# telegraphroad/VCNF

Measured on AMD Instinct MI355X. Metric: flow transforms/sec (log_prob + sample), D=64 RQ-spline, batch=1M, higher is better.
Workload: dtype f32 results on fp16x3 split operands: every fp32 operand of a conditioner GEMM travels as hi + lo fp16 halves, three f16 matrix instructions per product (four in the 48- and 16-deep layers), fp32 accumulation; measured against fp64 (tests/test_gpu_gemm_error.py): GEMM error 0.6-0.75x the exact-fp32

## Files before the change

### vcnf_amd/csrc/fused_layer_v6.hip

```cpp
#include <hip/hip_runtime.h>
#include <stdint.h>

#include "../../include/vcnf_hip.h"
#include "rqs_math.hpp"
#include "fused_common.hpp"
#include "host_common.hpp"
#include "rqs_lean.hpp"
#include "split_half.hpp"

#ifndef VCNF_ABL
#define VCNF_ABL 0
#endif
#ifndef VCNF_TIME
#define VCNF_TIME 0
#endif
#ifndef VCNF_AHEAD
#define VCNF_AHEAD 1
#endif
#if VCNF_TIME
#define VCNF_T(I) { const long long t_ = clock64(); tacc[I] += t_ - tlast; tlast = t_; }
#define VCNF_TIME_PARAM , float* tstamps
#define VCNF_TIME_ARG , time_buffer()
#else
#define VCNF_T(I)
#define VCNF_TIME_PARAM
#define VCNF_TIME_ARG
#endif

#define VCNF_SYNC() { __builtin_amdgcn_sched_barrier(0); asm volatile("s_waitcnt lgkmcnt(0)\n\ts_barrier" ::: "memory"); __builtin_amdgcn_sched_barrier(0); }

namespace vcnf {

#if VCNF_TIME
constexpr int kTimeSlots = 24;
static float* time_buffer() {
  static float* buf = nullptr;
  if (!buf && hipMalloc(&buf, 2 * kTimeSlots * sizeof(float)) != hipSuccess) buf = nullptr;
  return buf;
}
extern "C" int vcnf_v6_phase_stamps(float* out) {
  if (!time_buffer() || hipDeviceSynchronize() != hipSuccess) return VCNF_ERR_LAUNCH;
  return hipMemcpy(out, time_buffer(), 2 * kTimeSlots * sizeof(float), hipMemcpyDeviceToHost) == hipSuccess ? VCNF_OK : VCNF_ERR_LAUNCH;
}
#endif

template <int DI, int DT, int C, int H, int NBLK, int K, bool INV>
__global__ __launch_bounds__(512, 2) void fused_rqs_layer_v6_kernel(const FusedArgs a VCNF_TIME_PARAM) {
  static_assert(H == 128 && K == 8, "4 row blocks of 32 over 4 waves; 3 K - 1 = 23 logits: two features per 48 rows");
  static_assert((DI == 16 || DI == 32) && DT == DI && (C == 0 || C == 16), "shape family");
  constexpr int kBlock = 512;
  constexpr int kTile = 128;
  constexpr int NCB = 4;
  constexpr int D = DI + DT;
  constexpr int XS = D + 4;
  constexpr int NTX = DI / 16;
  constexpr int NTC = C / 16;
  constexpr int NT0 = NTX + NTC;
  constexpr int NTH = H / 16;
  constexpr int P = 3 * K - 1;
  constexpr int NG = DT / 4;
  constexpr int NR = NG / 2;
  constexpr int TABW = 3 * (K + 1);
  using L = PackLayout6<DI, DT, C, H, NBLK, K>;
  constexpr int GFRAG = 3 * NTH * 2 * 64;
  constexpr int RING = VCNF_AHEAD + 1;

  extern __shared__ __align__(16) float smem[];
  using S = LdsV6<DI, DT, C, H, NBLK, K>;
  static_assert(S::TILE == kTile && S::FRAG_N == 2 * GFRAG * 4 && S::XT_N == kTile * XS && S::TAB_N >= DI * TABW, "layout");
  uint4* act = reinterpret_cast<uint4*>(smem + S::FRAG);
  uint4* act_hi = act;
  uint4* act_lo = act + NTH * NCB * 64;
  float* xt = smem + S::XT;
  uint4* ctxf = reinterpret_cast<uint4*>(smem + S::CTXF);
  float* tab = smem + S::TAB;
  float* ldt = smem + S::LDT;
  int* tfi = reinterpret_cast<int*>(smem + S::TFI);
  int* idi = reinterpret_cast<int*>(smem + S::IDI);
  constexpr int NBV = C > 0 ? 3 : 2;
  constexpr int NBT = S::NBT;
  constexpr int BPL = S::BPL;
  float* biasf = smem + S::BIAS;
  float* ldold = smem + S::LDOLD;
  int* tflag = reinterpret_cast<int*>(smem + S::TFLAG);

  const int tid = threadIdx.x;
  const int lane = tid & 63;
  const int wave = __builtin_amdgcn_readfirstlane(tid >> 6);
  const int rp = wave & 3;
  const int ch = wave >> 2;
  const int c32 = lane & 31;
  const int kg = lane >> 5;
  const RqsConst& c = a.c;
  const bool shared = a.sh_w != nullptr;
  const LeanConst lc = make_lean_const(c);

  if (ch == 1) __builtin_amdgcn_s_setprio(1);
  for (int i = tid; i < NG * 96; i += kBlock) {
    const int g = i / 96, hf = i % 96 / 48;
    biasf[hf * BPL + g * 48 + i % 48] = a.wpack[L::BF + i];
  }
  for (int i = tid; i < NBT * H; i += kBlock) {
    const int v = i / H, blk = (v - 1) / NBV, sel = (v - 1) % NBV, r = i % H;
    const int off = v == 0 ? L::B0 : L::BLK0 + blk * L::BLK + (sel == 0 ? L::BA : sel == 1 ? L::BB : L::BC);
    biasf[(r >> 4 & 1) * BPL + NG * 48 + v * (H / 2) + (r >> 5) * 16 + (r & 15)] = a.wpack[off + r];
  }
  for (int i = tid; i < DT; i += kBlock) tfi[i] = a.tf_idx[i];
  for (int i = tid; i < DI; i += kBlock) idi[i] = a.id_idx[i];
  if (shared) {
    for (int i = tid; i < 3 * DI; i += kBlock) {
      const int f = i % DI;
      SplitLogits p{a.sh_w + f * K, a.sh_h + f * K, a.sh_d + f * (K - 1), K, 1.f, c.edge_logit, c.tails};
      rqs_build_table_part_k<K>(p, c, tab + f * TABW, 1, i / DI);
    }
  }

  const __amdgpu_buffer_rsrc_t wr =
      __builtin_amdgcn_make_buffer_rsrc(const_cast<float*>(a.wpack), 0, a.wpack_bytes, 0x00020000);
  const int voff = lane * 16;
  const float* bplane = biasf + kg * BPL;

  const long long ntiles = (a.B + kTile - 1) / kTile;
  bool bad = false;
  float satm = 0.f;
#if VCNF_TIME
  long long tacc[20], tlast = clock64();
  const long long tstart = tlast, rstart = wall_clock64();
  for (int i = 0; i < 20; ++i) tacc[i] = 0;
#endif
  float4 xpre[kTile * (D / 4) / kBlock], cpre[1];
  static_assert(kTile * (D / 4) % kBlock == 0 && (C == 0 || kTile * (C / 4) == kBlock), "rows per thread");
#define VCNF_PREFETCH_ROWS(TILE)                                                          \
  {                                                                                       \
    const long long pb0 = min((TILE) * kTile, a.B);                                       \
    const long long left = (a.B - pb0) * (D * 4);                                         \
    const __amdgpu_buffer_rsrc_t xr_ = __builtin_amdgcn_make_buffer_rsrc(                 \
        const_cast<float*>(a.x) + pb0 * D, 0, (int)min(left, (long long)(kTile * D * 4)), 0x00020000); \
    _Pragma("unroll") for (int k = 0; k < kTile * (D / 4) / kBlock; ++k)                  \
      xpre[k] = __builtin_bit_cast(float4, __builtin_amdgcn_raw_buffer_load_b128(xr_, (tid + kBlock * k) * 16, 0, 0)); \
    if (C > 0) {                                                                          \
      const long long leftc = (a.B - pb0) * (C * 4);                                      \
      const __amdgpu_buffer_rsrc_t cr_ = __builtin_amdgcn_make_buffer_rsrc(               \
          const_cast<float*>(a.ctx) + pb0 * C, 0, (int)min(leftc, (long long)(kTile * C * 4)), 0x00020000); \
      cpre[0] = __builtin_bit_cast(float4, __builtin_amdgcn_raw_buffer_load_b128(cr_, tid * 16, 0, 0)); \
    }                                                                                     \
  }
#define VCNF_ROWS_ARRIVED()                                                               \
  {                                                                                       \
    _Pragma("unroll") for (int k = 0; k < kTile * (D / 4) / kBlock; ++k) {                \
      floatx4 v_ = __builtin_bit_cast(floatx4, xpre[k]);                                  \
      asm volatile("" : "+v"(v_));                                                        \
      xpre[k] = __builtin_bit_cast(float4, v_);                                           \
    }                                                                                     \
    if (C > 0) {                                                                          \
      floatx4 v_ = __builtin_bit_cast(floatx4, cpre[0]);                                  \
      asm volatile("" : "+v"(v_));                                                        \
      cpre[0] = __builtin_bit_cast(float4, v_);                                           \
    }                                                                                     \
  }
  VCNF_PREFETCH_ROWS((long long)blockIdx.x)
  VCNF_ROWS_ARRIVED()
  for (long long tile = blockIdx.x; tile < ntiles; tile += gridDim.x) {
    const long long b0 = tile * kTile;
    const int rows = (int)min((long long)kTile, a.B - b0);
    satm = 0.f;
    { VCNF_T(0) VCNF_SYNC(); VCNF_T(15) }
    {
      constexpr int D4 = D / 4;
      if (tid == 0) *tflag = 0;
#pragma unroll
      for (int k = 0; k < kTile * D4 / kBlock; ++k) {
        const int i = tid + kBlock * k;
        const int r = i / D4, o = i - r * D4;
        *reinterpret_cast<float4*>(xt + r * XS + 4 * o) = xpre[k];
      }
      if (C > 0) {
        const int r = tid >> 2, part = tid & 3;
        half4 h4, l4;
        const float cv[4] = {cpre[0].x, cpre[0].y, cpre[0].z, cpre[0].w};
#pragma unroll
        for (int i = 0; i < 4; ++i) satm = fmaxf(satm, cv[i] == cv[i] ? __builtin_fabsf(cv[i]) : __builtin_inff());
        asm volatile("" : "+v"(satm));
#pragma unroll
        for (int i = 0; i < 4; ++i) {
          const float x = __builtin_amdgcn_fmed3f(cv[i], -65504.f, 65504.f);
          const _Float16 hv = (_Float16)x;
          h4[i] = hv;
          l4[i] = (_Float16)((x - (float)hv) * kLoScale);
        }
        const int at = (((r >> 5) * 2) * 64 + (r & 31) + 32 * (part >> 1));
        uint2* dh = reinterpret_cast<uint2*>(ctxf + at) + (part & 1);
        uint2* dl = reinterpret_cast<uint2*>(ctxf + at + 64) + (part & 1);
        *dh = __builtin_bit_cast(uint2, h4);
        *dl = __builtin_bit_cast(uint2, l4);
      }
    }
    { VCNF_T(1) VCNF_SYNC(); VCNF_T(15) }

    {
      constexpr int UNR = DI / 4;
      const int mi = tid >> 2, part = tid & 3;
      float lsum = 0.f;
      float xv[UNR], fv[UNR];
      float* px[UNR];
#pragma unroll
      for (int k = 0; k < UNR; ++k) {
        px[k] = xt + mi * XS + idi[part * UNR + k];
        xv[k] = *px[k];
        fv[k] = xv[k];
      }
      if (shared) {
        float yv[UNR], lad[UNR];
        bool in_[UNR];
#pragma unroll
        for (int k = 0; k < UNR; ++k) {
          in_[k] = (xv[k] >= c.lo_x) && (xv[k] <= c.hi_x);
          bool bad1 = false;
          rqs_point_table_inside<INV, K>(in_[k] ? xv[k] : c.lo_x, tab + (part * UNR + k) * TABW, yv[k], lad[k], bad1);
          bad = bad || (bad1 && in_[k]);
        }
#pragma unroll
        for (int k = 0; k < UNR; ++k) {
          const float o = in_[k] ? yv[k] : xv[k];
          *px[k] = o;
          if (INV) fv[k] = o;
          lsum += in_[k] ? lad[k] : 0.f;
        }
      }
      lsum += __shfl_xor(lsum, 1, 64);
      lsum += __shfl_xor(lsum, 2, 64);
      int tid_ = tid;
      asm volatile("" : "+v"(tid_));
      if (part == 0) ldt[tid_ >> 2] = lsum;
#pragma unroll
      for (int k = 0; k < UNR; ++k) satm = fmaxf(satm, fv[k] == fv[k] ? 0.f : __builtin_inff());
      const int k0 = part * UNR;
      const int t0 = k0 >> 4, kg0 = (k0 >> 3) & 1;
      const int at = (t0 * NCB + (mi >> 5)) * 64 + (mi & 31) + 32 * kg0;
      if (UNR == 8) {
        half8 h8, l8;
        float f8[8];
#pragma unroll
        for (int k = 0; k < 8; ++k) f8[k] = fv[k < UNR ? k : 0];
        split8<false>(f8, h8, l8, satm);
        act_hi[at] = __builtin_bit_cast(uint4, h8);
        act_lo[at] = __builtin_bit_cast(uint4, l8);
      } else {
        half4 h4, l4;
        satm = fmaxf(fmaxf(satm, __builtin_fabsf(fv[0])), __builtin_fabsf(fv[1]));
        satm = fmaxf(fmaxf(satm, __builtin_fabsf(fv[2 < UNR ? 2 : 0])), __builtin_fabsf(fv[3 < UNR ? 3 : 0]));
        asm volatile("" : "+v"(satm));
#pragma unroll
        for (int i = 0; i < 4; ++i) {
          const float x = __builtin_amdgcn_fmed3f(fv[i < UNR ? i : 0], -65504.f, 65504.f);
          const _Float16 hv = (_Float16)x;
          h4[i] = hv;
          l4[i] = (_Float16)((x - (float)hv) * kLoScale);
        }
        reinterpret_cast<uint2*>(act_hi + at)[(k0 >> 2) & 1] = __builtin_bit_cast(uint2, h4);
        reinterpret_cast<uint2*>(act_lo + at)[(k0 >> 2) & 1] = __builtin_bit_cast(uint2, l4);
      }
    }
    { VCNF_T(2) VCNF_SYNC(); VCNF_T(15) }
    if (ch == 1) { VCNF_T(14) VCNF_SYNC(); VCNF_T(16) }

    half8 ahi[NTH], alo[NTH];
    floatx16 abias;
#define VCNF_LOAD_BIAS16(DST, VEC)                                                        \
  _Pragma("unroll") for (int i_ = 0; i_ < 4; ++i_) {                                      \
    const floatx4 b4_ = *reinterpret_cast<const floatx4*>(bplane + NG * 48 + (VEC) * (H / 2) + 16 * rp + 4 * i_); \
    DST[4 * i_ + 0] = b4_[0]; DST[4 * i_ + 1] = b4_[1]; DST[4 * i_ + 2] = b4_[2]; DST[4 * i_ + 3] = b4_[3]; \
  }
#define VCNF_LOAD_HIDDEN(WOFF, BVEC)                                                      \
  {                                                                                       \
    _Pragma("unroll") for (int t = 0; t < NTH; ++t) {                                     \
      ahi[t] = __builtin_bit_cast(half8, wload(wr, voff, 4 * ((WOFF) + ((rp * NTH + t) * 2 + 0) * 256))); \
      alo[t] = __builtin_bit_cast(half8, wload(wr, voff, 4 * ((WOFF) + ((rp * NTH + t) * 2 + 1) * 256))); \
    }                                                                                     \
    VCNF_LOAD_BIAS16(abias, BVEC)                                                         \
  }

    floatx16 h[2];
    {
      half8 w0h[NT0], w0l[NT0];
      floatx16 bias0;
#pragma unroll
      for (int t = 0; t < NT0; ++t) {
        w0h[t] = __builtin_bit_cast(half8, wload(wr, voff, 4 * (L::W0 + ((rp * NT0 + t) * 2 + 0) * 256)));
        w0l[t] = __builtin_bit_cast(half8, wload(wr, voff, 4 * (L::W0 + ((rp * NT0 + t) * 2 + 1) * 256)));
      }
      VCNF_LOAD_BIAS16(bias0, 0)
#pragma unroll
      for (int j = 0; j < 2; ++j) {
        const int cb = 2 * ch + j;
        floatx16 mainv = bias0, corr = {}, corr2 = {};
#pragma unroll
        for (int t = 0; t < NT0; ++t) {
          const half8 bh = __builtin_bit_cast(half8, t < NTX ? act_hi[(t * NCB + cb) * 64 + lane] : ctxf[(cb * 2 + 0) * 64 + lane]);
          const half8 bl = __builtin_bit_cast(half8, t < NTX ? act_lo[(t * NCB + cb) * 64 + lane] : ctxf[(cb * 2 + 1) * 64 + lane]);
          mainv = mfma32h(w0h[t], bh, mainv);
          corr = mfma32h(w0h[t], bl, corr);
          corr = mfma32h(w0l[t], bh, corr);
          corr2 = mfma32h(w0l[t], bl, corr2);
        }
#pragma unroll
        for (int r = 0; r < 16; ++r) h[j][r] = fmaf(fmaf(corr2[r], kLoUnscale, corr[r]), kLoUnscale, mainv[r]);
      }
    }
    { VCNF_T(3) VCNF_SYNC(); VCNF_T(15) }
#define VCNF_PUBLISH(SRC, RELU)                                                           \
  _Pragma("unroll") for (int j = 0; j < 2; ++j) {                                         \
    _Pragma("unroll") for (int hh = 0; hh < 2; ++hh) {                                    \
      float v8_[8];                                                                       \
      _Pragma("unroll") for (int i = 0; i < 8; ++i) v8_[i] = SRC[j][8 * hh + i];          \
      half8 h8_, l8_;                                                                     \
      split8<RELU>(v8_, h8_, l8_, satm);                                                  \
      const int at = ((2 * rp + hh) * NCB + 2 * ch + j) * 64 + lane;                      \
      act_hi[at] = __builtin_bit_cast(uint4, h8_);                                        \
      act_lo[at] = __builtin_bit_cast(uint4, l8_);                                        \
    }                                                                                     \
  }
    VCNF_LOAD_HIDDEN(L::BLK0 + L::WA, 1)
    VCNF_PUBLISH(h, true)
    { VCNF_T(4) VCNF_SYNC(); VCNF_T(15) }

#define VCNF_READ_B(T)                                                                    \
  {                                                                                       \
    rh[(T) % RING] = __builtin_bit_cast(half8, act_hi[((((T) & 7)) * NCB + 2 * ch + ((T) >> 3)) * 64 + lane]); \
    rl[(T) % RING] = __builtin_bit_cast(half8, act_lo[((((T) & 7)) * NCB + 2 * ch + ((T) >> 3)) * 64 + lane]); \
  }
#define VCNF_HIDDEN_COMPUTE(OUT)                                                          \
  {                                                                                       \
    half8 rh[RING], rl[RING];                 \
    floatx16 corr;                                                                        \
    _Pragma("unroll") for (int st_ = 0; st_ < VCNF_AHEAD; ++st_) {                        \
      VCNF_READ_B(st_)                                                                    \
    }                                                                                     \
    _Pragma("unroll") for (int st_ = 0; st_ < 2 * NTH; ++st_) {                           \
      const int j = st_ >> 3, tk_ = st_ & 7;                                              \
      if (st_ + VCNF_AHEAD < 2 * NTH) {                                                   \
        VCNF_READ_B(st_ + VCNF_AHEAD)                                                     \
      }                                                                                   \
      if (tk_ == 0) {                                                                       \
        OUT[j] = abias;                                                                   \
        corr = floatx16{};                                                                \
      }                                                                                   \
      OUT[j] = mfma32h(ahi[tk_], rh[st_ % RING], OUT[j]);                                      \
      corr = mfma32h(ahi[tk_], rl[st_ % RING], corr);                                          \
      corr = mfma32h(alo[tk_], rh[st_ % RING], corr);                                          \
      if (tk_ == NTH - 1) {                                                                 \
        _Pragma("unroll") for (int r = 0; r < 16; ++r) OUT[j][r] = fmaf(corr[r], kLoUnscale, OUT[j][r]); \
      }                                                                                   \
    }                                                                                     \
    __builtin_amdgcn_sched_group_barrier(0x100, 2 * VCNF_AHEAD, 0);                       \
    _Pragma("unroll") for (int st_ = 0; st_ + VCNF_AHEAD < 2 * NTH; ++st_) {              \
      __builtin_amdgcn_sched_group_barrier(0x100, 2, 0);                                  \
      __builtin_amdgcn_sched_group_barrier(0x008, 3, 0);                                  \
    }                                                                                     \
    __builtin_amdgcn_sched_group_barrier(0x008, 3 * VCNF_AHEAD, 0);                       \
  }

#pragma unroll
    for (int blk = 0; blk < (VCNF_ABL == 5 ? 0 : NBLK); ++blk) {
      const int base = L::BLK0 + blk * L::BLK;
      floatx16 t[2];
      VCNF_HIDDEN_COMPUTE(t)
      { VCNF_T(5) VCNF_SYNC(); VCNF_T(15) }
      VCNF_LOAD_HIDDEN(base + L::WB, 2 + blk * NBV)
      half8 wch, wcl;
      floatx16 gate[2], gbias;
      if (C > 0) {
        wch = __builtin_bit_cast(half8, wload(wr, voff, 4 * (base + L::WC + (rp * 2 + 0) * 256)));
        wcl = __builtin_bit_cast(half8, wload(wr, voff, 4 * (base + L::WC + (rp * 2 + 1) * 256)));
        VCNF_LOAD_BIAS16(gbias, 3 + blk * NBV)
      }
      VCNF_PUBLISH(t, true)
      { VCNF_T(6) VCNF_SYNC(); VCNF_T(15) }
      VCNF_HIDDEN_COMPUTE(t)
      if (C > 0 && VCNF_ABL != 6) {
#pragma unroll
        for (int j = 0; j < 2; ++j) {
          const half8 bh = __builtin_bit_cast(half8, ctxf[((2 * ch + j) * 2 + 0) * 64 + lane]);
          const half8 bl = __builtin_bit_cast(half8, ctxf[((2 * ch + j) * 2 + 1) * 64 + lane]);
          floatx16 corr = {}, corr2 = {};
          gate[j] = mfma32h(wch, bh, gbias);
          corr = mfma32h(wch, bl, corr);
          corr = mfma32h(wcl, bh, corr);
          corr2 = mfma32h(wcl, bl, corr2);
#pragma unroll
          for (int r = 0; r < 16; ++r) gate[j][r] = fmaf(fmaf(corr2[r], kLoUnscale, corr[r]), kLoUnscale, gate[j][r]);
        }
      }
      { VCNF_T(5) VCNF_SYNC(); VCNF_T(15) }
      if (blk + 1 < NBLK) {
        VCNF_LOAD_HIDDEN(base + L::BLK + L::WA, 1 + (blk + 1) * NBV)
      }
      if (C > 0 && VCNF_ABL != 6) {
#pragma unroll
        for (int j = 0; j < 2; ++j) {
#pragma unroll
          for (int r = 0; r < 16; ++r) {
            const float sg = hw_rcp(1.f + hw_exp2(-gate[j][r]));
            h[j][r] = fmaf(t[j][r], sg, h[j][r]);
          }
        }
      } else {
#pragma unroll
        for (int j = 0; j < 2; ++j) h[j] += t[j];
      }
      if (blk + 1 < NBLK) {
        VCNF_PUBLISH(h, true)
      } else {
        VCNF_PUBLISH(h, false)
      }
      { VCNF_T(7) VCNF_SYNC(); VCNF_T(15) }
    }
    if (ch == 0) { VCNF_T(14) VCNF_SYNC(); VCNF_T(17) }
#undef VCNF_HIDDEN_COMPUTE
#undef VCNF_READ_B
#undef VCNF_LOAD_HIDDEN
#undef VCNF_PUBLISH

    half8 fhi[NTH], flo[NTH];
#pragma unroll
    for (int t = 0; t < NTH; ++t) {
      fhi[t] = __builtin_bit_cast(half8, act_hi[(t * NCB + rp) * 64 + lane]);
      flo[t] = __builtin_bit_cast(half8, act_lo[(t * NCB + rp) * 64 + lane]);
    }
    float ld_acc = 0.f;
    uint4* win = act + ch * GFRAG;
    const int gtid = tid & 255;
    constexpr int NSTG = GFRAG / 256;
    static_assert(GFRAG % 256 == 0, "whole fragments per thread");
#define VCNF_STAGE_DMA(G)                                                                 \
  _Pragma("unroll") for (int k = 0; k < NSTG; ++k)                                        \
    dma16_to_lds(wr, win + (gtid & ~63) + k * 256, gtid * 16, 4 * (L::WF + (G) * (4 * GFRAG) + k * 1024));
    floatx16 pa[3];
#define VCNF_LOAD_BIASF(G)                                                                \
  _Pragma("unroll") for (int b = 0; b < 3; ++b) {                                         \
    _Pragma("unroll") for (int i_ = 0; i_ < 4; ++i_) {                                    \
      const floatx4 b4_ = *reinterpret_cast<const floatx4*>(bplane + (G) * 48 + 16 * b + 4 * i_); \
      pa[b][4 * i_ + 0] = b4_[0]; pa[b][4 * i_ + 1] = b4_[1]; pa[b][4 * i_ + 2] = b4_[2]; pa[b][4 * i_ + 3] = b4_[3]; \
    }                                                                                     \
  }
    VCNF_LOAD_BIASF(ch)
    { VCNF_T(8) VCNF_SYNC(); VCNF_T(15) }
    VCNF_STAGE_DMA(ch)
    if (ch == 0 && rp < 2 && a.ld_mode) {
      const __amdgpu_buffer_rsrc_t or_ = __builtin_amdgcn_make_buffer_rsrc(a.logdet + b0, 0, rows * 4, 0x00020000);
      __builtin_amdgcn_raw_ptr_buffer_load_lds(or_, (__attribute__((address_space(3))) void*)(ldold + rp * 64), 4,
                                               lane * 4, rp * 256, 0, 0);
    }
    wait_vector_memory();
    { VCNF_T(9) VCNF_SYNC(); VCNF_T(15) }
    if (ch == 1) { VCNF_T(14) VCNF_SYNC(); VCNF_T(18) }
    for (int rnd = 0; rnd < (VCNF_ABL == 3 ? 0 : NR); ++rnd) {
      const int g = 2 * rnd + ch;
      float* px[2];
      float xin[2];
#pragma unroll
      for (int f2 = 0; f2 < 2; ++f2) {
        px[f2] = xt + (rp * 32 + c32) * XS + tfi[4 * g + 2 * kg + f2];
        xin[f2] = *px[f2];
      }
      {
        half8 wh[RING], wl[RING];
        floatx16 corr;
#define VCNF_READ_W(T)                                                                    \
  {                                                                                       \
    wh[(T) % RING] = __builtin_bit_cast(half8, win[((T) * 2 + 0) * 64 + lane]);           \
    wl[(T) % RING] = __builtin_bit_cast(half8, win[((T) * 2 + 1) * 64 + lane]);           \
  }
#pragma unroll
        for (int u = 0; u < VCNF_AHEAD; ++u) {
          VCNF_READ_W(u)
        }
#pragma unroll
        for (int u = 0; u < 3 * NTH; ++u) {
          const int b = u >> 3, t = u & 7;
          if (u + VCNF_AHEAD < 3 * NTH) {
            VCNF_READ_W(u + VCNF_AHEAD)
          }
          if (t == 0) corr = floatx16{};
          pa[b] = mfma32h(wh[u % RING], fhi[t], pa[b]);
          corr = mfma32h(wh[u % RING], flo[t], corr);
          corr = mfma32h(wl[u % RING], fhi[t], corr);
          if (t == NTH - 1) {
#pragma unroll
            for (int r = 0; r < 16; ++r) pa[b][r] = fmaf(corr[r], kLoUnscale, pa[b][r]);
          }
        }
        __builtin_amdgcn_sched_group_barrier(0x100, 2 * VCNF_AHEAD, 0);
#pragma unroll
        for (int u = 0; u + VCNF_AHEAD < 3 * NTH; ++u) {
          __builtin_amdgcn_sched_group_barrier(0x100, 2, 0);
          __builtin_amdgcn_sched_group_barrier(0x008, 3, 0);
        }
        __builtin_amdgcn_sched_group_barrier(0x008, 3 * VCNF_AHEAD, 0);
#undef VCNF_READ_W
      }
      { VCNF_T(10) VCNF_SYNC(); VCNF_T(15) }
      {
        const bool more = rnd + 1 < NR;
        if (!more) {
          VCNF_PREFETCH_ROWS(tile + gridDim.x)
        }
        if (more && VCNF_ABL != 2) {
          VCNF_STAGE_DMA(g + 2)
        }
        float yv[2], lad[2];
#pragma unroll
        for (int f2 = 0; f2 < 2; ++f2) {
          float lg[P];
#pragma unroll
          for (int tl = 0; tl < P; ++tl) lg[tl] = pa[(24 * f2 + tl) >> 4][(24 * f2 + tl) & 15];
          rqs_lean_eval<8, INV>(xin[f2], lg, lc, yv[f2], lad[f2], bad);
        }
        *px[0] = yv[0];
        *px[1] = yv[1];
        ld_acc += lad[0] + lad[1];
        if (more) {
          VCNF_LOAD_BIASF(g + 2)
        }
      }
      if (rnd + 1 < NR && VCNF_ABL != 2) wait_vector_memory();
      { VCNF_T(11) VCNF_SYNC(); VCNF_T(15) }
    }
    if (ch == 0) { VCNF_T(14) VCNF_SYNC(); VCNF_T(19) }
#undef VCNF_PREFETCH_ROWS
#undef VCNF_STAGE_DMA
#undef VCNF_LOAD_BIASF

    ld_acc += __shfl_xor(ld_acc, 32, 64);
    if (ch == 1 && kg == 0) ldt[rp * 32 + c32] += ld_acc;
    if (satm > 65504.f) *tflag = 1;
    { VCNF_T(12) VCNF_SYNC(); VCNF_T(15) }
    VCNF_ROWS_ARRIVED()
#undef VCNF_ROWS_ARRIVED
    int tid_ = tid;
    asm volatile("" : "+v"(tid_));
    const bool over = *tflag != 0;
    if (tid == 0 && over && a.sat) atomicAdd(a.sat, 1);
    if (a.redo) {
      if (tid_ < kTile / kFusedFlagRows) {
        const __amdgpu_buffer_rsrc_t rr = __builtin_amdgcn_make_buffer_rsrc(
            a.redo + tile * (kTile / kFusedFlagRows), 0, 4 * ((rows + kFusedFlagRows - 1) / kFusedFlagRows), 0x00020000);
        __builtin_amdgcn_raw_buffer_store_b32(over ? 1 : 0, rr, tid_ * 4, 0, 0);
      }
      if (over) continue;
    }
    if (ch == 0 && (tid_ & 32) == 0) {
      const int mrow = (tid_ >> 6) * 32 + (tid_ & 31);
      const __amdgpu_buffer_rsrc_t lr = __builtin_amdgcn_make_buffer_rsrc(a.logdet + b0, 0, rows * 4, 0x00020000);
      const float o = a.ld_sign * (ld_acc + ldt[mrow]);
      __builtin_amdgcn_raw_buffer_store_b32(__builtin_bit_cast(unsigned, a.ld_mode ? ldold[mrow] + o : o), lr, mrow * 4, 0, 0);
    }
    {
      constexpr int D4 = D / 4;
      const __amdgpu_buffer_rsrc_t yr = __builtin_amdgcn_make_buffer_rsrc(a.y + b0 * D, 0, rows * (D * 4), 0x00020000);
      floatx4 yv[kTile * D4 / kBlock];
#pragma unroll
      for (int k = 0; k < kTile * D4 / kBlock; ++k) {
        const int i = tid_ + kBlock * k;
        const int r = i / D4, o = i - r * D4;
        yv[k] = *reinterpret_cast<const floatx4*>(xt + r * XS + 4 * o);
      }
#pragma unroll
      for (int k = 0; k < kTile * D4 / kBlock; ++k)
        __builtin_amdgcn_raw_buffer_store_b128(__builtin_bit_cast(__attribute__((ext_vector_type(4))) unsigned, yv[k]), yr, (tid_ + kBlock * k) * 16, 0, 0);
    }
  }
#if VCNF_TIME
  VCNF_T(13)
  if (blockIdx.x == 0 && (tid & 255) == 0 && tstamps) {
    float* ts = tstamps + (tid >> 8) * kTimeSlots;
    for (int i = 0; i < 20; ++i) ts[i] = (float)tacc[i];
    ts[20] = (float)(clock64() - tstart);
    ts[21] = (float)(wall_clock64() - rstart);
    ts[22] = (float)((ntiles - blockIdx.x + gridDim.x - 1) / gridDim.x);
  }
#endif
  if (INV && a.bad && bad) atomicAdd(a.bad, 1);
}

template <int DI, int DT, int C, int H, int NBLK, int K>
static int launch_v6(const FusedArgs& a, int inverse, hipStream_t st) {
  constexpr int TILE = 128;
  constexpr size_t lds = LdsV6<DI, DT, C, H, NBLK, K>::BYTES;
  const bool set = inverse ? lds_limit_once<&fused_rqs_layer_v6_kernel<DI, DT, C, H, NBLK, K, true>>(lds)
                           : lds_limit_once<&fused_rqs_layer_v6_kernel<DI, DT, C, H, NBLK, K, false>>(lds);
  if (!set) return VCNF_ERR_LAUNCH;
  const long long ntiles = (a.B + TILE - 1) / TILE;
  dim3 grid((unsigned)(ntiles < 256 ? ntiles : 256));
  if (inverse)
    hipLaunchKernelGGL((fused_rqs_layer_v6_kernel<DI, DT, C, H, NBLK, K, true>), grid, dim3(512), lds, st, a VCNF_TIME_ARG);
  else
    hipLaunchKernelGGL((fused_rqs_layer_v6_kernel<DI, DT, C, H, NBLK, K, false>), grid, dim3(512), lds, st, a VCNF_TIME_ARG);
  return launched();
}

template <int NBLK>
static int launch_v6_family(const FusedArgs& a, int d_id, int ctx_dim, int inverse, hipStream_t st) {
#ifdef VCNF_DEV_ONLY
  return launch_v6<32, 32, 16, 128, NBLK, 8>(a, inverse, st);
#else
  return with_fused_shape(d_id, ctx_dim,
                          [&](auto DI, auto C) { return launch_v6<DI(), DI(), C(), 128, NBLK, 8>(a, inverse, st); });
#endif
}

#ifndef VCNF_V6_NBLK
#define VCNF_V6_NBLK 2
#endif
VCNF_BLOCKS_ENTRY(launch_fused_v6_b, VCNF_V6_NBLK, FusedArgs, launch_v6_family)

}
```

### vcnf_amd/csrc/fused_lds.hpp

```cpp
#pragma once

#include <stddef.h>

namespace vcnf {

template <int DI, int DT, int C, int H, int NBLK, int K>
struct LdsV6 {
  static constexpr int TILE = 128, D = DI + DT, NG = DT / 4;
  static constexpr int NBT = 1 + NBLK * (C > 0 ? 3 : 2);
  static constexpr int BPL = NG * 48 + NBT * (H / 2);
  static constexpr int FRAG = 0, FRAG_N = 2 * 3 * (H / 16) * 2 * 64 * 4;
  static constexpr int XT = FRAG + FRAG_N, XT_N = TILE * (D + 4);
  static constexpr int CTXF = XT + XT_N, CTXF_N = C > 0 ? 4 * 2 * 64 * 4 : 0;
  static constexpr int TAB = CTXF + CTXF_N, TAB_N = (DI * 3 * (K + 1) + 3) & ~3;
  static constexpr int LDT = TAB + TAB_N, LDT_N = TILE;
  static constexpr int TFI = LDT + LDT_N, TFI_N = DT;
  static constexpr int IDI = TFI + TFI_N, IDI_N = DI + 4;
  static constexpr int BIAS = IDI + IDI_N, BIAS_N = 2 * BPL;
  static constexpr int LDOLD = BIAS + BIAS_N, LDOLD_N = TILE;
  static constexpr int TFLAG = LDOLD + LDOLD_N, TFLAG_N = 1;
  static constexpr int END = TFLAG + TFLAG_N;
  static constexpr size_t SLACK_BYTES = 3 * 4 + 64;
  static constexpr size_t BYTES = (size_t)END * 4 + SLACK_BYTES;
  static_assert(FRAG == 0 && FRAG + FRAG_N <= XT && XT + XT_N <= CTXF && CTXF + CTXF_N <= TAB && TAB + TAB_N <= LDT &&
                    LDT + LDT_N <= TFI && TFI + TFI_N <= IDI && IDI + IDI_N <= BIAS && BIAS + BIAS_N <= LDOLD &&
                    LDOLD + LDOLD_N <= TFLAG && (size_t)(TFLAG + TFLAG_N) * 4 <= BYTES,
                "regions in order, none overlaps the next, the last ends within BYTES");
  static_assert(XT % 4 == 0 && CTXF % 4 == 0 && TAB % 4 == 0, "16-byte aligned rows and fragments");
};

template <int DI, int DT, int C, int H, int NBLK, int K>
struct LdsV6s {
  static constexpr int TILE = 32, D = DI + DT, NG = DT / 4;
  static constexpr int TABF = (DI * 3 * (K + 1) + 3) & ~3;
  static constexpr int TSET = TABF + DT + DI + 4 + NG * 96;
  static constexpr int ACT = 0, ACT_N = 4 * (H / 16) * 64 * 4;
  static constexpr int XT = ACT + ACT_N, XT_N = TILE * (D + 4);
  static constexpr int CTXF = XT + XT_N, CTXF_N = C > 0 ? 2 * 64 * 4 : 0;
  static constexpr int LDT = CTXF + CTXF_N, LDT_N = TILE;
  static constexpr int LDX = LDT + LDT_N, LDX_N = 8 * TILE;
  static constexpr int TFLAG = LDX + LDX_N, TFLAG_N = 4;
  static constexpr int TSETS = TFLAG + TFLAG_N, TSETS_N = 2 * TSET;
  static constexpr int END = TSETS + TSETS_N;
  static constexpr size_t SLACK_BYTES = 64;
  static constexpr size_t BYTES = (size_t)END * 4 + SLACK_BYTES;
  static_assert(ACT == 0 && ACT + ACT_N <= XT && XT + XT_N <= CTXF && CTXF + CTXF_N <= LDT && LDT + LDT_N <= LDX &&
                    LDX + LDX_N <= TFLAG && TFLAG + TFLAG_N <= TSETS && (size_t)(TSETS + TSETS_N) * 4 <= BYTES,
                "regions in order, none overlaps the next, the last ends within BYTES");
  static_assert(XT % 4 == 0 && CTXF % 4 == 0 && TSETS % 4 == 0 && TSET % 4 == 0, "16-byte aligned rows and tables");
};

template <int DI, int DT, int C, int H, int NBLK, int K, int kCB>
struct LdsF32 {
  static constexpr int TILE = 4 * kCB * 16, D = DI + DT;
  static constexpr int XT = 0, XT_N = TILE * (D + 4);
  static constexpr int CT = XT + XT_N, CT_N = TILE * ((C > 0 ? C : 4) + 4);
  static constexpr int TAB = CT + CT_N, TAB_N = (DI * 3 * (K + 1) + 3) & ~3;
  static constexpr int TFI = TAB + TAB_N, TFI_N = DT;
  static constexpr int IDI = TFI + TFI_N, IDI_N = DI;
  static constexpr int END = IDI + IDI_N;
  static constexpr size_t SLACK_BYTES = 64;
  static constexpr size_t BYTES = (size_t)END * 4 + SLACK_BYTES;
  static_assert(XT + XT_N <= CT && CT + CT_N <= TAB && TAB + TAB_N <= TFI && TFI + TFI_N <= IDI &&
                    (size_t)(IDI + IDI_N) * 4 <= BYTES,
                "regions in order, none overlaps the next, the last ends within BYTES");
  static_assert(CT % 4 == 0 && TAB % 4 == 0, "16-byte aligned rows");
};

}
```

### vcnf_amd/csrc/rqs_math.hpp

```cpp
#pragma once
#include <hip/hip_runtime.h>
#include <math.h>

#include "rqs_host.hpp"

#pragma clang fp contract(off)

namespace vcnf {

constexpr float kLog2e = 1.44269504088896340736f;
constexpr float kLn2 = 0.69314718055994530942f;
__device__ __forceinline__ float hw_exp2(float v) { return __builtin_amdgcn_exp2f(v); }
__device__ __forceinline__ float hw_rcp(float v) { return __builtin_amdgcn_rcpf(v); }
__device__ __forceinline__ float hw_log(float v) { return __builtin_amdgcn_logf(v) * kLn2; }
__device__ __forceinline__ float hw_sqrt(float v) { return __builtin_amdgcn_sqrtf(v); }
__device__ __forceinline__ float div_nr(float a, float b) {
  const float r = hw_rcp(b);
  const float q = a * r;
  return fmaf(fmaf(-b, q, a), r, q);
}

__device__ __forceinline__ float softplus_f(float v) {
  const float e = hw_exp2(v * kLog2e);
  const float u = 1.f + e;
  const float um1 = u - 1.f;
  const float l = (um1 == 0.f) ? e : hw_log(u) * div_nr(e, um1);
  return v > 20.f ? v : l;
}

__device__ __forceinline__ float rqs_rounding_level_zero(float disc, float qb, float p) {
  const float scale = fmaf(qb, qb, __builtin_fabsf(p));
  return (disc < 0.f && disc >= -6.103515625e-5f * scale) ? 0.f : disc;
}

struct RqsBin {
  float xl, w, yl, h, d0, d1;
};

template <bool INV>
__device__ __forceinline__ void rqs_bin_eval(float x, const RqsBin& b, float& y, float& lad, bool& bad) {
  const float s = div_nr(b.h, b.w);
  const float e = fmaf(-2.f, s, b.d0 + b.d1);
  if (!INV) {
    const float t = div_nr(x - b.xl, b.w);
    const float omt = 1.f - t;
    const float tt = t * omt;
    const float num = b.h * fmaf(s * t, t, b.d0 * tt);
    const float den = fmaf(e, tt, s);
    y = b.yl + div_nr(num, den);
    const float dn = (s * s) * fmaf(b.d1 * t, t, fmaf(2.f * s, tt, (b.d0 * omt) * omt));
    lad = fmaf(-2.f, hw_log(den), hw_log(dn));
  } else {
    const float dy = x - b.yl;
    const float qa = fmaf(dy, e, b.h * (s - b.d0));
    const float qb = fmaf(-dy, e, b.h * b.d0);
    const float qc = -s * dy;
    const float fa = 4.f * qa;
    const float p = fa * qc;
    const float perr = fmaf(fa, qc, -p);
    const float disc = rqs_rounding_level_zero(fmaf(qb, qb, -p) - perr, qb, p);
    bad = bad || !(disc >= 0.f);
    float r = div_nr(2.f * qc, -qb - hw_sqrt(disc));
    r = (dy <= b.h && r > 1.f) ? 1.f : r;
    y = fmaf(r, b.w, b.xl);
    const float omr = 1.f - r;
    const float rr = r * omr;
    const float den = fmaf(e, rr, s);
    const float dn = (s * s) * fmaf(b.d1 * r, r, fmaf(2.f * s, rr, (b.d0 * omr) * omr));
    lad = fmaf(2.f, hw_log(den), -hw_log(dn));
  }
}

template <int KT, bool INV, class P>
__device__ __forceinline__ void rqs_select(float x, const P& p, const RqsConst& c, float sc2, RqsBin& sel) {
  const int K = KT > 0 ? KT : c.K;
  constexpr int KR = KT > 0 ? KT : 1;
  float ew[KR], eh[KR];
  float mw = -INFINITY, mh = -INFINITY;
#pragma unroll
  for (int k = 0; k < K; ++k) {
    mw = fmaxf(mw, p.w(k));
    mh = fmaxf(mh, p.h(k));
  }
  float sw = 0.f, sh = 0.f;
#pragma unroll
  for (int k = 0; k < K; ++k) {
    const float a = hw_exp2((p.w(k) - mw) * sc2), b = hw_exp2((p.h(k) - mh) * sc2);
    if (KT > 0) { ew[k] = a; eh[k] = b; }
    sw += a;
    sh += b;
  }
  const float gw = div_nr(c.free_w, sw), gh = div_nr(c.free_h, sh);
  float cw = 0.f, ch = 0.f;
  float xl = c.lo_x, yl = c.lo_y, dl = p.d(0);
  sel.xl = xl; sel.yl = yl; sel.w = 1.f; sel.h = 1.f; sel.d0 = dl; sel.d1 = dl;
#pragma unroll
  for (int k = 0; k < K; ++k) {
    const float a = KT > 0 ? ew[k] : hw_exp2((p.w(k) - mw) * sc2);
    const float b = KT > 0 ? eh[k] : hw_exp2((p.h(k) - mh) * sc2);
    cw += fmaf(a, gw, c.min_w);
    ch += fmaf(b, gh, c.min_h);
    const float xr = (k == K - 1) ? c.hi_x : fmaf(c.span_x, cw, c.lo_x);
    const float yr = (k == K - 1) ? c.hi_y : fmaf(c.span_y, ch, c.lo_y);
    const float dr = p.d(k + 1);
    const bool take = (k == 0) || (INV ? (x >= yl) : (x >= xl));
    if (take) {
      sel.xl = xl; sel.w = xr - xl;
      sel.yl = yl; sel.h = yr - yl;
      sel.d0 = dl; sel.d1 = dr;
    }
    xl = xr; yl = yr; dl = dr;
  }
  sel.d0 = c.min_d + softplus_f(sel.d0);
  sel.d1 = c.min_d + softplus_f(sel.d1);
}

template <int K, bool INV>
struct RqsStaged {
  float ew[K], eh[K];
  float mw, mh, sw, sh, gw, gh, cw, ch, xl, yl, dl;
  RqsBin sel;
  template <class P>
  __device__ __forceinline__ void maxima(const P& p) {
    mw = -INFINITY;
    mh = -INFINITY;
#pragma unroll
    for (int k = 0; k < K; ++k) {
      mw = fmaxf(mw, p.w(k));
      mh = fmaxf(mh, p.h(k));
    }
    sw = 0.f;
    sh = 0.f;
  }
  template <class P>
  __device__ __forceinline__ void exps(const P& p, float sc2, int k0, int k1) {
#pragma unroll
    for (int k = 0; k < K; ++k) {
      if (k >= k0 && k < k1) {
        ew[k] = hw_exp2((p.w(k) - mw) * sc2);
        eh[k] = hw_exp2((p.h(k) - mh) * sc2);
        sw += ew[k];
        sh += eh[k];
      }
    }
  }
  template <class P>
  __device__ __forceinline__ void normalise(const P& p, const RqsConst& c) {
    gw = div_nr(c.free_w, sw);
    gh = div_nr(c.free_h, sh);
    cw = 0.f;
    ch = 0.f;
    xl = c.lo_x;
    yl = c.lo_y;
    dl = p.d(0);
    sel.xl = xl; sel.yl = yl; sel.w = 1.f; sel.h = 1.f; sel.d0 = dl; sel.d1 = dl;
  }
  template <class P>
  __device__ __forceinline__ void knots(float x, const P& p, const RqsConst& c, int k0, int k1) {
#pragma unroll
    for (int k = 0; k < K; ++k) {
      if (k < k0 || k >= k1) continue;
      cw += fmaf(ew[k], gw, c.min_w);
      ch += fmaf(eh[k], gh, c.min_h);
      const float xr = (k == K - 1) ? c.hi_x : fmaf(c.span_x, cw, c.lo_x);
      const float yr = (k == K - 1) ? c.hi_y : fmaf(c.span_y, ch, c.lo_y);
      const float dr = p.d(k + 1);
      const bool take = (k == 0) || (INV ? (x >= yl) : (x >= xl));
      sel.xl = take ? xl : sel.xl;
      sel.w = take ? xr - xl : sel.w;
      sel.yl = take ? yl : sel.yl;
      sel.h = take ? yr - yl : sel.h;
      sel.d0 = take ? dl : sel.d0;
      sel.d1 = take ? dr : sel.d1;
      xl = xr; yl = yr; dl = dr;
    }
  }
  __device__ __forceinline__ void derivatives(const RqsConst& c) {
    sel.d0 = c.min_d + softplus_f(sel.d0);
    sel.d1 = c.min_d + softplus_f(sel.d1);
  }
};

template <int KT, bool INV, class P>
__device__ __forceinline__ void rqs_point(float x, const P& p, const RqsConst& c,
                                          float& y, float& lad, bool& bad) {
  if (c.tails != 0 && !((x >= c.lo_x) && (x <= c.hi_x))) {
    y = x;
    lad = 0.f;
    return;
  }
  RqsBin sel;
  rqs_select<KT, INV>(x, p, c, p.scale * kLog2e, sel);
  rqs_bin_eval<INV>(x, sel, y, lad, bad);
}

struct PackedLogits {
  const float* q;
  int K;
  float scale, edge;
  int tails;
  __device__ __forceinline__ float w(int k) const { return q[k]; }
  __device__ __forceinline__ float h(int k) const { return q[K + k]; }
  __device__ __forceinline__ float d(int k) const {
    if (tails == 1) return (k == 0 || k == K) ? edge : q[2 * K + k - 1];
    if (tails == 2) return q[2 * K + (k == K ? 0 : k)];
    return q[2 * K + k];
  }
};

struct SplitLogits {
  const float *pw, *ph, *pd;
  int K;
  float scale, edge;
  int tails;
  __device__ __forceinline__ float w(int k) const { return pw[k]; }
  __device__ __forceinline__ float h(int k) const { return ph[k]; }
  __device__ __forceinline__ float d(int k) const {
    if (tails == 1) return (k == 0 || k == K) ? edge : pd[k - 1];
    if (tails == 2) return pd[k == K ? 0 : k];
    return pd[k];
  }
};

struct StridedLogits {
  const float *pw, *ph, *pd;
  long long ks;
  int K;
  float scale, edge;
  int tails;
  __device__ __forceinline__ float w(int k) const { return pw[k * ks]; }
  __device__ __forceinline__ float h(int k) const { return ph[k * ks]; }
  __device__ __forceinline__ float d(int k) const {
    if (tails == 1) return (k == 0 || k == K) ? edge : pd[(k - 1) * ks];
    if (tails == 2) return pd[(k == K ? 0 : k) * ks];
    return pd[k * ks];
  }
};

template <class P>
__device__ __forceinline__ void rqs_build_table_part(const P& p, const RqsConst& c, float* tab, int stride, int part) {
  const int K = c.K;
  float* col = tab + part * (K + 1) * stride;
  if (part == 2) {
    for (int k = 0; k <= K; ++k) col[k * stride] = c.min_d + softplus_f(p.d(k));
    return;
  }
  const bool xs = part == 0;
  float m = -INFINITY;
  for (int k = 0; k < K; ++k) m = fmaxf(m, xs ? p.w(k) : p.h(k));
  const float sc2 = p.scale * kLog2e;
  float sum = 0.f;
  for (int k = 0; k < K; ++k) sum += hw_exp2(((xs ? p.w(k) : p.h(k)) - m) * sc2);
  const float g = div_nr(xs ? c.free_w : c.free_h, sum);
  const float mn = xs ? c.min_w : c.min_h, span = xs ? c.span_x : c.span_y, lo = xs ? c.lo_x : c.lo_y;
  float cum = 0.f;
  col[0] = lo;
  for (int k = 0; k < K; ++k) {
    cum += fmaf(hw_exp2(((xs ? p.w(k) : p.h(k)) - m) * sc2), g, mn);
    col[(k + 1) * stride] = (k == K - 1) ? (xs ? c.hi_x : c.hi_y) : fmaf(span, cum, lo);
  }
}

template <int K, class P>
__device__ __forceinline__ void rqs_table_column_load(const P& p, int part, float (&v)[K + 1]) {
#pragma unroll
  for (int k = 0; k <= K; ++k) v[k] = part == 2 ? p.d(k) : (k < K ? (part == 0 ? p.w(k) : p.h(k)) : 0.f);
}

template <int K>
__device__ __forceinline__ void rqs_table_column_build(const float (&v)[K + 1], float scale, const RqsConst& c, float* tab,
                                                       int stride, int part) {
  float* col = tab + part * (K + 1) * stride;
  if (part == 2) {
#pragma unroll
    for (int k = 0; k <= K; ++k) col[k * stride] = c.min_d + softplus_f(v[k]);
    return;
  }
  const bool xs = part == 0;
  float e[K];
  float m = -INFINITY;
#pragma unroll
  for (int k = 0; k < K; ++k) m = fmaxf(m, v[k]);
  const float sc2 = scale * kLog2e;
  float sum = 0.f;
#pragma unroll
  for (int k = 0; k < K; ++k) {
    e[k] = hw_exp2((v[k] - m) * sc2);
    sum += e[k];
  }
  const float g = div_nr(xs ? c.free_w : c.free_h, sum);
  const float mn = xs ? c.min_w : c.min_h, span = xs ? c.span_x : c.span_y, lo = xs ? c.lo_x : c.lo_y;
  float cum = 0.f;
  col[0] = lo;
#pragma unroll
  for (int k = 0; k < K; ++k) {
    cum += fmaf(e[k], g, mn);
    col[(k + 1) * stride] = (k == K - 1) ? (xs ? c.hi_x : c.hi_y) : fmaf(span, cum, lo);
  }
}

template <int K, class P>
__device__ __forceinline__ void rqs_build_table_part_k(const P& p, const RqsConst& c, float* tab, int stride, int part) {
  float v[K + 1];
  rqs_table_column_load<K>(p, part, v);
  rqs_table_column_build<K>(v, p.scale, c, tab, stride, part);
}

template <class P>
__device__ __forceinline__ void rqs_build_table(const P& p, const RqsConst& c, float* tab, int stride = 1) {
#pragma unroll 1
  for (int part = 0; part < 3; ++part) rqs_build_table_part(p, c, tab, stride, part);
}

template <bool INV, int KT = 0>
__device__ __forceinline__ void rqs_point_table(float x, const float* tab, const RqsConst& c,
                                                float& y, float& lad, bool& bad) {
  if (c.tails != 0 && !((x >= c.lo_x) && (x <= c.hi_x))) {
    y = x;
    lad = 0.f;
    return;
  }
  const int K = KT > 0 ? KT : c.K;
  const float* xk = tab;
  const float* yk = tab + (K + 1);
  const float* dk = tab + 2 * (K + 1);
  int bin = 0;
  const float* key = INV ? yk : xk;
  if (KT > 0) {
#pragma unroll
    for (int k = 1; k < KT; ++k) bin += (x >= key[k]) ? 1 : 0;
  } else {
    for (int k = 1; k < K; ++k) bin += (x >= key[k]) ? 1 : 0;
  }
  RqsBin b;
  b.xl = xk[bin];
  b.w = xk[bin + 1] - b.xl;
  b.yl = yk[bin];
  b.h = yk[bin + 1] - b.yl;
  b.d0 = dk[bin];
  b.d1 = dk[bin + 1];
  rqs_bin_eval<INV>(x, b, y, lad, bad);
}

template <bool INV, int KT>
__device__ __forceinline__ void rqs_point_table_inside(float x, const float* tab, float& y, float& lad, bool& bad) {
  const float* xk = tab;
  const float* yk = tab + (KT + 1);
  const float* dk = tab + 2 * (KT + 1);
  const float* key = INV ? yk : xk;
  int bin = 0;
#pragma unroll
  for (int k = 1; k < KT; ++k) bin += (x >= key[k]) ? 1 : 0;
  RqsBin b;
  b.xl = xk[bin];
  b.w = xk[bin + 1] - b.xl;
  b.yl = yk[bin];
  b.h = yk[bin + 1] - b.yl;
  b.d0 = dk[bin];
  b.d1 = dk[bin + 1];
  rqs_bin_eval<INV>(x, b, y, lad, bad);
}

}
```

Before: 68.98 million.

## Precompute per-bin spline records in LDS and binary-search bins for shared RQS

Once per block, builds an 8-float record per spline bin (width reciprocal, slope, derivative terms, and inverse-quadratic coefficients) in an LDS region appended after the existing layout. The per-point evaluation then finds the bin with a branchless binary search across all unrolled points instead of a linear scan, loads the record with two float4 reads, and evaluates with fewer divides. The intent is to cut per-point ALU and LDS scalar loads in the shared-table spline stage. The cost is extra LDS per block, which may reduce occupancy, plus an added barrier and setup work at kernel start.

```diff
diff --git a/vcnf_amd/csrc/fused_layer_v6.hip b/vcnf_amd/csrc/fused_layer_v6.hip
--- a/vcnf_amd/csrc/fused_layer_v6.hip
+++ b/vcnf_amd/csrc/fused_layer_v6.hip
@@ -67,13 +67,15 @@
 
   extern __shared__ __align__(16) float smem[];
   using S = LdsV6<DI, DT, C, H, NBLK, K>;
-  static_assert(S::TILE == kTile && S::FRAG_N == 2 * GFRAG * 4 && S::XT_N == kTile * XS && S::TAB_N >= DI * TABW, "layout");
+  static_assert(S::TILE == kTile && S::FRAG_N == 2 * GFRAG * 4 && S::XT_N == kTile * XS && S::TAB_N >= DI * TABW &&
+                    S::BINS_PART == (DI / 4) * K * kRqsBinRec + 4 && S::BINS_N == 4 * S::BINS_PART, "layout");
   uint4* act = reinterpret_cast<uint4*>(smem + S::FRAG);
   uint4* act_hi = act;
   uint4* act_lo = act + NTH * NCB * 64;
   float* xt = smem + S::XT;
   uint4* ctxf = reinterpret_cast<uint4*>(smem + S::CTXF);
   float* tab = smem + S::TAB;
+  float* bins = smem + S::BINS;
   float* ldt = smem + S::LDT;
   int* tfi = reinterpret_cast<int*>(smem + S::TFI);
   int* idi = reinterpret_cast<int*>(smem + S::IDI);
@@ -113,6 +115,9 @@
       SplitLogits p{a.sh_w + f * K, a.sh_h + f * K, a.sh_d + f * (K - 1), K, 1.f, c.edge_logit, c.tails};
       rqs_build_table_part_k<K>(p, c, tab + f * TABW, 1, i / DI);
     }
+    VCNF_SYNC();
+    for (int i = tid; i < DI * K; i += kBlock)
+      rqs_build_bin_record<INV, K>(tab + (i / K) * TABW, i % K, bins + i * kRqsBinRec + (i / (DI / 4 * K)) * 4);
   }
 
   const __amdgpu_buffer_rsrc_t wr =
@@ -212,11 +217,27 @@
       if (shared) {
         float yv[UNR], lad[UNR];
         bool in_[UNR];
+        int part_ = part;
+        asm volatile("" : "+v"(part_));
+        const float* ftab = tab + part_ * (UNR * TABW);
+        const float* brec = bins + part_ * S::BINS_PART;
+        float xin[UNR];
+        const float* key[UNR];
+        int bin[UNR];
 #pragma unroll
         for (int k = 0; k < UNR; ++k) {
           in_[k] = (xv[k] >= c.lo_x) && (xv[k] <= c.hi_x);
+          xin[k] = in_[k] ? xv[k] : c.lo_x;
+          key[k] = ftab + k * TABW + (INV ? K + 1 : 0);
+        }
+        rqs_bin_search_n<K, UNR>(xin, key, bin);
+        RqsBinPoint<INV, K> bp[UNR];
+#pragma unroll
+        for (int k = 0; k < UNR; ++k) bp[k].load(bin[k], ftab + k * TABW, brec + k * (K * kRqsBinRec));
+#pragma unroll
+        for (int k = 0; k < UNR; ++k) {
           bool bad1 = false;
-          rqs_point_table_inside<INV, K>(in_[k] ? xv[k] : c.lo_x, tab + (part * UNR + k) * TABW, yv[k], lad[k], bad1);
+          bp[k].eval(xin[k], yv[k], lad[k], bad1);
           bad = bad || (bad1 && in_[k]);
         }
 #pragma unroll
@@ -586,7 +607,7 @@
 template <int DI, int DT, int C, int H, int NBLK, int K>
 static int launch_v6(const FusedArgs& a, int inverse, hipStream_t st) {
   constexpr int TILE = 128;
-  constexpr size_t lds = LdsV6<DI, DT, C, H, NBLK, K>::BYTES;
+  constexpr size_t lds = LdsV6<DI, DT, C, H, NBLK, K>::LAUNCH_BYTES;
   const bool set = inverse ? lds_limit_once<&fused_rqs_layer_v6_kernel<DI, DT, C, H, NBLK, K, true>>(lds)
                            : lds_limit_once<&fused_rqs_layer_v6_kernel<DI, DT, C, H, NBLK, K, false>>(lds);
   if (!set) return VCNF_ERR_LAUNCH;
diff --git a/vcnf_amd/csrc/fused_lds.hpp b/vcnf_amd/csrc/fused_lds.hpp
--- a/vcnf_amd/csrc/fused_lds.hpp
+++ b/vcnf_amd/csrc/fused_lds.hpp
@@ -3,6 +3,8 @@
 #include <stddef.h>
 
 namespace vcnf {
+
+constexpr size_t kLdsPerCu = 160 * 1024;
 
 template <int DI, int DT, int C, int H, int NBLK, int K>
 struct LdsV6 {
@@ -27,6 +29,10 @@
                     LDOLD + LDOLD_N <= TFLAG && (size_t)(TFLAG + TFLAG_N) * 4 <= BYTES,
                 "regions in order, none overlaps the next, the last ends within BYTES");
   static_assert(XT % 4 == 0 && CTXF % 4 == 0 && TAB % 4 == 0, "16-byte aligned rows and fragments");
+  static constexpr int BINS_PART = (DI / 4) * K * 8 + 4;
+  static constexpr int BINS = (int)((BYTES + 15) / 16) * 4, BINS_N = 4 * BINS_PART;
+  static constexpr size_t LAUNCH_BYTES = (size_t)(BINS + BINS_N) * 4;
+  static_assert((size_t)BINS * 4 >= BYTES && BINS % 4 == 0 && LAUNCH_BYTES <= kLdsPerCu, "appended region: behind BYTES, 16-byte aligned, within the compute unit");
 };
 
 template <int DI, int DT, int C, int H, int NBLK, int K>
diff --git a/vcnf_amd/csrc/rqs_math.hpp b/vcnf_amd/csrc/rqs_math.hpp
--- a/vcnf_amd/csrc/rqs_math.hpp
+++ b/vcnf_amd/csrc/rqs_math.hpp
@@ -361,4 +361,114 @@
   rqs_bin_eval<INV>(x, b, y, lad, bad);
 }
 
-}
+constexpr int kRqsBinRec = 8;
+
+template <bool INV, int KT>
+__device__ __forceinline__ void rqs_build_bin_record(const float* tab, int bin, float* rec) {
+  const float* xk = tab;
+  const float* yk = tab + (KT + 1);
+  const float* dk = tab + 2 * (KT + 1);
+  RqsBin b;
+  b.xl = xk[bin];
+  b.w = xk[bin + 1] - b.xl;
+  b.yl = yk[bin];
+  b.h = yk[bin + 1] - b.yl;
+  b.d0 = dk[bin];
+  b.d1 = dk[bin + 1];
+  const float s = div_nr(b.h, b.w);
+  const float e = fmaf(-2.f, s, b.d0 + b.d1);
+  if (!INV) {
+    rec[0] = b.xl; rec[1] = b.w; rec[2] = hw_rcp(b.w); rec[3] = b.h;
+    rec[4] = s; rec[5] = e; rec[6] = b.d0; rec[7] = b.d1;
+  } else {
+    rec[0] = b.yl; rec[1] = e; rec[2] = b.h * (s - b.d0); rec[3] = b.h * b.d0;
+    rec[4] = s; rec[5] = b.h; rec[6] = b.w; rec[7] = b.xl;
+  }
+}
+
+template <int KT, int N>
+__device__ __forceinline__ void rqs_bin_search_n(const float (&x)[N], const float* const (&key)[N], int (&bin)[N]) {
+#pragma unroll
+  for (int i = 0; i < N; ++i) bin[i] = 0;
+  if ((KT & (KT - 1)) == 0) {
+#pragma unroll
+    for (int step = KT / 2; step >= 1; step >>= 1) {
+      float kv[N];
+#pragma unroll
+      for (int i = 0; i < N; ++i) kv[i] = key[i][bin[i] + step];
+#pragma unroll
+      for (int i = 0; i < N; ++i) bin[i] += (x[i] >= kv[i]) ? step : 0;
+    }
+  } else {
+#pragma unroll
+    for (int i = 0; i < N; ++i) {
+#pragma unroll
+      for (int k = 1; k < KT; ++k) bin[i] += (x[i] >= key[i][k]) ? 1 : 0;
+    }
+  }
+}
+
+template <bool INV, int KT>
+struct RqsBinPoint {
+  float4 ra, rb;
+  float g0, g1;
+  __device__ __forceinline__ void load(int bin, const float* tab, const float* recs) {
+    ra = *reinterpret_cast<const float4*>(recs + bin * kRqsBinRec);
+    rb = *reinterpret_cast<const float4*>(recs + bin * kRqsBinRec + 4);
+    g0 = tab[(INV ? 2 : 1) * (KT + 1) + bin];
+    g1 = INV ? tab[2 * (KT + 1) + bin + 1] : 0.f;
+  }
+  __device__ __forceinline__ void eval(float x, float& y, float& lad, bool& bad) const;
+};
+
+template <bool INV, int KT>
+__device__ __forceinline__ void RqsBinPoint<INV, KT>::eval(float x, float& y, float& lad, bool& bad) const {
+  if (!INV) {
+    const float xl = ra.x, w = ra.y, rw = ra.z, h = ra.w, s = rb.x, e = rb.y, d0 = rb.z, d1 = rb.w;
+    const float yl = g0;
+    const float a = x - xl;
+    const float q = a * rw;
+    const float t = fmaf(fmaf(-w, q, a), rw, q);
+    const float omt = 1.f - t;
+    const float tt = t * omt;
+    const float num = h * fmaf(s * t, t, d0 * tt);
+    const float den = fmaf(e, tt, s);
+    y = yl + div_nr(num, den);
+    const float dn = (s * s) * fmaf(d1 * t, t, fmaf(2.f * s, tt, (d0 * omt) * omt));
+    lad = fmaf(-2.f, hw_log(den), hw_log(dn));
+  } else {
+    const float yl = ra.x, e = ra.y, ha = ra.z, hb = ra.w, s = rb.x, h = rb.y, w = rb.z, xl = rb.w;
+    const float d0 = g0, d1 = g1;
+    const float dy = x - yl;
+    const float qa = fmaf(dy, e, ha);
+    const float qb = fmaf(-dy, e, hb);
+    const float qc = -s * dy;
+    const float fa = 4.f * qa;
+    const float p = fa * qc;
+    const float perr = fmaf(fa, qc, -p);
+    const float disc = rqs_rounding_level_zero(fmaf(qb, qb, -p) - perr, qb, p);
+    bad = bad || !(disc >= 0.f);
+    float r = div_nr(2.f * qc, -qb - hw_sqrt(disc));
+    r = (dy <= h && r > 1.f) ? 1.f : r;
+    y = fmaf(r, w, xl);
+    const float omr = 1.f - r;
+    const float rr = r * omr;
+    const float den = fmaf(e, rr, s);
+    const float dn = (s * s) * fmaf(d1 * r, r, fmaf(2.f * s, rr, (d0 * omr) * omr));
+    lad = fmaf(2.f, hw_log(den), -hw_log(dn));
+  }
+}
+
+template <bool INV, int KT>
+__device__ __forceinline__ void rqs_point_bins_inside(float x, const float* tab, const float* recs, float& y, float& lad,
+                                                      bool& bad) {
+  const float xs[1] = {x};
+  const float* const key[1] = {INV ? tab + (KT + 1) : tab};
+  int bin[1];
+  rqs_bin_search_n<KT, 1>(xs, key, bin);
+  RqsBinPoint<INV, KT> p;
+  p.load(bin[0], tab, recs);
+  p.eval(x, y, lad, bad);
+}
+
+}
```

After: 69.59 million (median of 6 runs). No clear change (+0.9%).
